# JGI-Bioinformatics/Kmernator

Hardware: AMD Instinct MI355X
Metric: total k-mers/sec at k=31, 150 bp reads (spectrum build, inputs resident in HBM) (higher is better)
Workload: dtype u64

## Files before the change

### kmernator_amd/csrc/kmr_api.hip

```cpp
#include <hip/hip_runtime.h>
#include <dlfcn.h>
#include <unistd.h>
#include <rccl/rccl.h>

#include <algorithm>
#include <atomic>
#include <cmath>
#include <cstdio>
#include <cstdlib>
#include <cstring>
#include <cctype>
#include <memory>
#include <mutex>
#include <string>
#include <type_traits>
#include <vector>

#include "kmr_host.hpp"
#include "kmr_kernels.hpp"
#include "kmr_partition.hpp"
#include "kmr_superkmer.hpp"
#include "kmr_buckets.hpp"
#include "kmr_synth.hpp"
#define KMR_INSTANCES_EXTERN
// ... 1453 lines not shown
		uint32_t dv[2] = {SK_UNI_NONE, 0u};
		HIPCHK(h, hipMemcpy(dv, h->d_uni.get<uint32_t>(), 8, hipMemcpyDeviceToHost));
		if (dv[1]) mixed = true;
		else if (dv[0] != SK_UNI_NONE) { if (w == SK_UNI_NONE) w = dv[0]; else if (w != dv[0]) mixed = true; }
	}
	if (!mixed && w != SK_UNI_NONE) { uni = true; uni_wbits = w; }
	return 0;
}
template <int W> SkLong<W> sk_own_lists(kmr_handle *h, bool refined) {
	SkLong<W> lg{};
	lg.list_first = 0; lg.list_stride = 1;
	if (h->sk_exchange && h->cfg.world_size > 1 && !refined) { lg.list_first = h->cfg.rank; lg.list_stride = h->cfg.world_size; }
	return lg;
}
template <int W> struct SkCountLaunch {
	void (*kern)(PoolView, const uint64_t *, const uint64_t *, uint64_t, uint32_t, CountOut, FinalizeParams, unsigned int *, uint32_t, SkTrackView, SkLong<W>);
	size_t smem;
};
template <int W, int LOG2S, bool TRACK, bool EXT, bool UNI> SkCountLaunch<W> sk_count_form() { return {sk_count_kernel<W, LOG2S, TRACK, EXT, UNI>, sk_count_smem_bytes<W, LOG2S, TRACK, EXT, UNI>()}; }
template <int W> int sk_count_select(kmr_handle *h, bool ext, bool tracking, bool uni, SkCountLaunch<W> &k) {
	k = ext ? sk_count_form<W, COUNT_LOG2S_EXT, false, true, false>() : (tracking ? sk_count_form<W, COUNT_LOG2S, true, false, false>() :
	    (uni ? sk_count_form<W, COUNT_LOG2S, false, false, true>() : sk_count_form<W, COUNT_LOG2S, false, false, false>()));
	const auto kern = k.kern; const size_t smem = k.smem;
	HIPCHK(h, hipFuncSetAttribute((const void *)kern, hipFuncAttributeMaxDynamicSharedMemorySize, (int)smem));
	return 0;
}

template <int W> struct SkFinalize : CountPass {
	bool tracking = false, refined = false, uni = false;
	uint64_t nl = 1; uint64_t *ls = nullptr, *lc = nullptr; uint32_t nch = 0;
	SkTrackView tv{};
	SkLong<W> lgMain{}, lgItems{}; uint64_t n_items = 0;
	uint64_t early_slots = 0; FinalizeCounters early_c{};
};

int sk_refine_lists(kmr_handle *h, uint64_t &nl) {
	const uint32_t fine_bits = h->sk_bits + h->sk_fine_shift;
	const uint64_t nlf = 1ull << fine_bits;
	unsigned int head = 0;
// ... 87 lines not shown
	else { out.wkeys = h->uw_keys.get<uint64_t>(); out.wvals = h->uw_vals.get<uint32_t>(); out.wcap = key_entries(h, h->uw_keys); out.spkt = h->us_pkt.get<uint32_t>(); out.weakCount = wc; }
	out.wcursor = cursors; out.scursor = cursors + 1;
	out.skeys = h->us_keys.get<uint64_t>(); out.sweight = h->us_b8.get<uint8_t>(); out.scap = key_entries(h, h->us_keys);
	out.singCount = sc; out.fc = fc; out.err = h->derr.get<uint32_t>();
	return out;
}
template <int W> int sk_count_pass(kmr_handle *h, SkFinalize<W> &p) {
	const uint64_t nl = p.nl, n_items = p.n_items; const SkTrackView &tv = p.tv;
	uint32_t merge_log2 = 16;
	DevBuf mslots, mext;
	return count_attempts(h, p, [&]() -> int { mslots.reset(); mext.reset(); return 0; }, [&](const CountOut &out, bool repeated, uint32_t &repeat_on) -> int {
		if (repeated) merge_log2 += 3;
		int rc = 0;
		const int grid = (int)std::min<uint64_t>((uint64_t)num_cus(h) * 4, (nl / p.lgMain.list_stride + SK_LBATCH) / SK_LBATCH);
		SkCountLaunch<W> k;
		rc = sk_count_select<W>(h, p.ext, p.tracking, p.uni, k); if (rc) return rc;
		if (p.tracking) HIPCHK(h, hipMemsetAsync(tv.d_unique, 0, 8 * (tv.n + 1), h->stream));
		if (dbg()) { int nb = 0; hipOccupancyMaxActiveBlocksPerMultiprocessor(&nb, (const void *)k.kern, SKC_THREADS, k.smem); fprintf(stderr, "sk_count<W=%d>: %d blocks per CU (LDS %zu), %llu lists, %u chunks\n", W, nb, k.smem, (unsigned long long)nl, p.nch); }
		hipLaunchKernelGGL(k.kern, dim3(grid), dim3(SKC_THREADS), k.smem, h->stream, pool_view(h, h->l1), p.ls, p.lc, nl, h->k, out, p.f, h->work_counter.get<unsigned int>(), sk_dbg_flags("KMR_SK_COUNT_DBG"), tv, p.lgMain);
		HIPCHK(h, hipGetLastError());
		if (!n_items) return 0;
		SkLong<W> &lgItems = p.lgItems;
		if (mslots.alloc(sizeof(Slot<W>) << merge_log2) != hipSuccess) return fail(h, KMR_ERR_OOM, "merge table of the long lists");
		if (p.ext && mext.alloc(sizeof(ExtSlot) << merge_log2) != hipSuccess) return fail(h, KMR_ERR_OOM, "merge table of the long lists");
		hipLaunchKernelGGL(table_clear_kernel<W>, dim3(grid_for(1ull << merge_log2)), dim3(256), 0, h->stream, mslots.get<Slot<W>>(), mext.get<ExtSlot>(), 1ull << merge_log2);
		lgItems.merge.slots = mslots.get<Slot<W>>(); lgItems.merge.ext = mext.get<ExtSlot>(); lgItems.merge.log2cap = merge_log2;
		HIPCHK(h, hipMemsetAsync(lgItems.merge_used, 0, 8, h->stream));
		rc = zero_work_counter(h); if (rc) return rc;
		const int grid2 = (int)std::min<uint64_t>((uint64_t)num_cus(h) * 4, n_items);
		hipLaunchKernelGGL(k.kern, dim3(grid2), dim3(SKC_THREADS), k.smem, h->stream, pool_view(h, h->l1), p.ls, p.lc, nl, h->k, out, p.f, h->work_counter.get<unsigned int>(), sk_dbg_flags("KMR_SK_COUNT_DBG"), tv, lgItems);
		hipLaunchKernelGGL(sk_merge_emit_kernel<W>, dim3(grid_for(1ull << merge_log2)), dim3(256), 0, h->stream, lgItems.merge, out, p.f);
		if (hipGetLastError() != hipSuccess) return fail(h, KMR_ERR_HIP, "long-list launches");
		if (merge_log2 < 30) repeat_on = ERR_TABLE_FULL;
		return 0;
	});
}
template <int W> int sk_append_early(kmr_handle *h, SkFinalize<W> &p) {
	FinalizeCounters &c = p.c; const FinalizeCounters &early_c = p.early_c; unsigned long long *cur = p.cur; const uint64_t early_slots = p.early_slots;
	const size_t eb = 8ull * (W + 1);
	if (cur[0] + early_slots > packed_entries(h, h->ue)) {
		DevBuf bigger;
		HIPCHK(h, bigger.alloc(eb * (cur[0] + early_slots + 4096)));
		HIPCHK(h, hipMemcpyAsync(bigger.get(), h->ue.get(), eb * cur[0], hipMemcpyDeviceToDevice, h->stream)); HIPCHK(h, hipStreamSynchronize(h->stream));
		h->ue = std::move(bigger);
	}
// ... 89 lines not shown
	const SkTrackView tv{};
	SkLong<W> lg = sk_own_lists<W>(h, false);
	lg.long_threshold = h->tune.long_list_chunks ? h->tune.long_list_chunks : 1024;
	uint32_t *sc = nullptr;
	rc = arena_get(h, &sc, h->nb_sing); if (rc) return rc;
	HIPCHK(h, hipMemsetAsync(sc, 0, 4 * h->nb_sing, h->stream));
	CountOut out{};
	out.wentries = h->early.ue.get<uint64_t>(); out.wcursor = h->early.cursor.get<unsigned long long>(); out.wcap = packed_entries(h, h->early.ue);
	out.scursor = h->early.cursor.get<unsigned long long>() + 1;
	out.singCount = sc; out.fc = (FinalizeCounters *)h->early.fc.get(); out.err = h->early.err.get<uint32_t>();
	rc = zero_work_counter(h); if (rc) return rc;
	const uint64_t n_work = hi > lg.list_first ? (hi - lg.list_first + lg.list_stride - 1) / lg.list_stride : 0;
	if (n_work) {
		const int grid = (int)std::min<uint64_t>((uint64_t)num_cus(h) * 4, (n_work + SK_LBATCH) / SK_LBATCH);
		SkCountLaunch<W> k;
		rc = sk_count_select<W>(h, false, false, uni, k); if (rc) return rc;
		TimeSpan t(h, KMR_TIME_COUNT);
		hipLaunchKernelGGL(k.kern, dim3(grid), dim3(SKC_THREADS), k.smem, h->stream, pool_view(h, h->l1), ls, lc, hi, h->k, out, f, h->work_counter.get<unsigned int>(), sk_dbg_flags("KMR_SK_COUNT_DBG"), tv, lg);
		t.end();
		HIPCHK(h, hipGetLastError());
	}
	h->early.active = true; h->early.hi = hi; h->early.min_depth = min_depth;
	return KMR_OK;
}
int count_prefix_superkmer(kmr_handle *h, uint32_t min_depth, uint64_t hi) { return with_w(h, [&](auto W) { return count_prefix_superkmer_t<W()>(h, min_depth, hi); }); }
int finalize_superkmer(kmr_handle *h, uint32_t min_depth) { return with_w(h, [&](auto W) { return finalize_superkmer_t<W()>(h, min_depth); }); }

template <class M> void release(kmr_handle *h) { static_cast<M &>(*h) = M(); }

void free_partition_state(kmr_handle *h) {
	release<BuildMem>(h);
	if (h->tb_copy_stream) { hipStreamDestroy(h->tb_copy_stream); h->tb_copy_stream = nullptr; for (int a = 0; a < 2; a++) { hipEventDestroy(h->tb_ready[a]); hipEventDestroy(h->tb_consumed[a]); h->tb_set_used[a] = false; } }
}

// ... 1226 lines not shown
```

### kmernator_amd/csrc/kmr_instances.hpp

```cpp
#ifndef KMR_INSTANCES_HPP_
#define KMR_INSTANCES_HPP_

#include "kmr_superkmer.hpp"

namespace kmr {

static const int COUNT_LOG2S = 10;
static const int COUNT_LOG2S_EXT = 9;
static const int PD_THREADS = 1024, PD_RPT = 8, PD_LINE = 4;

#ifdef KMR_INSTANCES_EXTERN
#define KMR_T extern template
#else
#define KMR_T template
#endif

#define KMR_SKX(W, WIN, FILT) KMR_T __global__ void sk_extract_kernel<W, WIN, FILT, false>(ReadsView, DevParams, SkParams, PoolView); KMR_T __global__ void sk_extract_kernel<W, WIN, FILT, true>(ReadsView, DevParams, SkParams, PoolView);
#define KMR_SKXL(W, WIN) KMR_T __global__ void sk_extract_lean_kernel<W, WIN, false>(ReadsView, DevParams, SkParams, PoolView, float, SkPacked); KMR_T __global__ void sk_extract_lean_kernel<W, WIN, true>(ReadsView, DevParams, SkParams, PoolView, float, SkPacked);
#define KMR_SKX_W(W) KMR_SKX(W, 16, false) KMR_SKX(W, 16, true) KMR_SKX(W, 8, false) KMR_SKX(W, 8, true) KMR_SKX(W, 4, false) KMR_SKX(W, 4, true) KMR_SKXL(W, 16) KMR_SKXL(W, 8) KMR_SKXL(W, 4)

#define KMR_SKX_W32(W) KMR_SKX(W, 32, false) KMR_SKX(W, 32, true) KMR_SKXL(W, 32)

#define KMR_SKC(W, TRACK) KMR_SKCX(W, TRACK, false)
#define KMR_SKCX(W, TRACK, EXT) KMR_T __global__ void sk_count_kernel<W, EXT ? COUNT_LOG2S_EXT : COUNT_LOG2S, TRACK, EXT>(PoolView, const uint64_t *, const uint64_t *, uint64_t, uint32_t, CountOut, FinalizeParams, unsigned int *, uint32_t, SkTrackView, SkLong<W>);
#define KMR_SKL(W) KMR_T __global__ void sk_lookup_kernel<W>(PoolView, const uint64_t *, const uint64_t *, uint64_t, uint32_t, const uint64_t *, const uint64_t *, const uint32_t *, uint32_t *, uint64_t, unsigned int *, const uint64_t *, const uint64_t *, const uint32_t *, uint64_t, uint64_t);
#define KMR_SKCU(W) KMR_T __global__ void sk_count_kernel<W, COUNT_LOG2S, false, false, true>(PoolView, const uint64_t *, const uint64_t *, uint64_t, uint32_t, CountOut, FinalizeParams, unsigned int *, uint32_t, SkTrackView, SkLong<W>);
#define KMR_SKC_W(W) KMR_SKC(W, false) KMR_SKCU(W) KMR_SKC(W, true) KMR_SKCX(W, false, true) KMR_SKL(W)

#define KMR_EX(W, EXT, OP, SUB) KMR_T __global__ void extract_kernel<W, EXT, OP, SUB>(ReadsView, DevParams, OP);
#define KMR_EX_OP(W, EXT, ...) KMR_T __global__ void extract_kernel<W, EXT, __VA_ARGS__, false>(ReadsView, DevParams, __VA_ARGS__); KMR_T __global__ void extract_kernel<W, EXT, __VA_ARGS__, true>(ReadsView, DevParams, __VA_ARGS__);
#define KMR_EX_W(W) \
	KMR_EX_OP(W, false, InsertOp<W, false>) KMR_EX_OP(W, true, InsertOp<W, true>) \
	KMR_EX_OP(W, false, LinearOp<W, false, false>) KMR_EX_OP(W, false, LinearOp<W, false, true>) \
	KMR_EX_OP(W, true, LinearOp<W, true, false>) KMR_EX_OP(W, true, LinearOp<W, true, true>) \
	KMR_T __global__ void extract_kernel<W, false, LookupOp<W>, false>(ReadsView, DevParams, LookupOp<W>); \
	KMR_T __global__ void extract_kernel<W, false, LookupWeightOp<W>, false>(ReadsView, DevParams, LookupWeightOp<W>);

#define KMR_PD(W, EXT, LEVEL) KMR_T __global__ void partition_direct_kernel<W, EXT, LEVEL, PD_THREADS, PD_RPT, PD_LINE>(PartSource<W>, PoolView, unsigned int *, const int, const int);
#define KMR_OS(W, EXT, REQ) KMR_T __global__ void owner_scatter_kernel<W, EXT, REQ>(const typename PoolRec<W, EXT>::type *, const uint64_t *, const uint32_t *, uint64_t, uint32_t, uint32_t, uint32_t *, uint64_t, unsigned long long *, unsigned int *, uint32_t *, uint32_t *, OwnerFn);
#define KMR_CK(W, EXT, LOG2S, NARROW) KMR_T __global__ void count_kernel<W, EXT, LOG2S, NARROW>(PoolView, const uint64_t *, const uint64_t *, uint64_t, CountOut, FinalizeParams, unsigned int *, int);
#define KMR_PART_W(W) \
	KMR_PD(W, false, 1) KMR_PD(W, false, 2) KMR_PD(W, true, 1) KMR_PD(W, true, 2) \
// ... 34 lines not shown
```

### kmernator_amd/csrc/kmr_superkmer.hpp

```cpp
#ifndef KMR_SUPERKMER_HPP_
#define KMR_SUPERKMER_HPP_

#include "kmr_partition.hpp"
#include "kmr_buckets.hpp"

namespace kmr {

#ifndef KMR_SK_MAX_N
#define KMR_SK_MAX_N 128
#endif
static const uint32_t SK_CHUNK_G = 64;
static const uint32_t SK_MAX_N = KMR_SK_MAX_N;
static const int SK_WAVES = 3;
static const int SK_WINDOW = 16;
static const int SK_RR = 3, SKL_RR = 4;

#ifdef KMR_DEBUG_HOOKS
#define SK_DBG(flags, bit) (((flags) & (bit)) != 0)
#else
#define SK_DBG(flags, bit) false
#endif
struct SkTrackRec { uint32_t raw, good; unsigned long long end_ordinal; };
static const uint32_t SK_TRACK_MAX = 512;
struct SkTrackView { const unsigned long long *bounds; uint32_t n; unsigned int *d_unique, *d_single; };
// ... 1209 lines not shown

static const int SK_STAGE_CHUNKS = 4;
static const int SK_STAGE_G = SK_STAGE_CHUNKS * SK_CHUNK_G;
static const uint32_t SK_LBATCH = 24;
static const uint32_t SK_DESC_CAP = 160;

template <int W> struct SkLong {
	const uint64_t *item_c0, *item_c1;
	uint64_t n_items;
	uint64_t long_threshold;
	uint32_t list_first, list_stride;
	Table<W> merge;
	unsigned long long *merge_used;
};

template <int W, int LOG2S, bool TRACK = false, bool EXT = false, bool UNI = false>
__host__ __device__ constexpr size_t sk_count_smem_bytes() { return (size_t)(1 << LOG2S) * (8 * W + 24 + (W > 1 ? 4 : 0) - (UNI && W > 1 ? 12 : 0) + (TRACK ? 8 : 0) + (EXT ? 28 : 0)) + (size_t)SK_STAGE_G * 16 + 256 + 64 + (TRACK ? 8 * (SK_TRACK_MAX + 1) : 0); }
static const uint64_t SK_EXT_LONG_CHUNKS = 128;
static const int SK_EXT_BLOCKS = 3;
__device__ __forceinline__ uint32_t sk_ext_char(uint32_t code) { return (uint32_t)((0x584e54474341ull >> (8 * code)) & 0xffu); }

#ifndef KMR_SKC_WAVES
#define KMR_SKC_WAVES 4
#endif
static const int SKC_WAVES = KMR_SKC_WAVES, SKC_THREADS = SKC_WAVES * 64;
static const unsigned long long SK_KEY_PENDING = ~0ull;
static const uint32_t SK_ORDERED_FROM = 256;
static const unsigned long long SK_OSLAB = 2048;

template <int W, int LOG2S, bool TRACK = false, bool EXT = false, bool UNI = false>
__global__ __launch_bounds__(SKC_THREADS, EXT ? (W == 1 ? (LOG2S <= 9 ? SK_EXT_BLOCKS : 2) : 1) : ((W == 1 && LOG2S <= 10 && !TRACK) ? 4 : (W == 2 && LOG2S <= 10 && !TRACK ? (UNI ? 4 : 3) : 1)))
void sk_count_kernel(PoolView pool, const uint64_t *list_start, const uint64_t *list_chunks, uint64_t n_lists, uint32_t k,
                     CountOut out, FinalizeParams f, unsigned int *work_counter, uint32_t dbgFlags, SkTrackView tv, SkLong<W> lg) {
	static_assert(!UNI || (!TRACK && !EXT), "the one-weight count pass is the plain one's");
	constexpr int S = 1 << LOG2S;
	constexpr bool LEAN = UNI && W > 1;
#ifndef KMR_SKC_LIMIT_PCT
#define KMR_SKC_LIMIT_PCT 80
#endif
	constexpr uint32_t LIMIT = (uint32_t)(S * (KMR_SKC_LIMIT_PCT / 100.0));
	constexpr int WSLOTS = S / SKC_WAVES;
	extern __shared__ __attribute__((aligned(16))) uint8_t csm[];
	uint64_t *tkeys = (uint64_t *)csm;
	unsigned long long *tcnt = (unsigned long long *)(tkeys + (size_t)S * W);
	double *twsum = (double *)(tcnt + S);
	unsigned long long *tfirst = (unsigned long long *)(twsum + (LEAN ? 0 : S));
	uint32_t *tstate = (uint32_t *)(tfirst + S);
	uint32_t *ttally = tstate + (W > 1 && !LEAN ? S : 0);
	uint32_t *tpkt = ttally + (EXT ? 6 * S : 0);
	uint4 *stage = (uint4 *)(tpkt + (EXT ? S : 0));
	uint8_t *recOf = (uint8_t *)(stage + SK_STAGE_G);
	unsigned long long *tsecond = (unsigned long long *)(csm + (size_t)S * (8 * W + 24 + (W > 1 ? 4 : 0) + (EXT ? 28 : 0)) + (size_t)SK_STAGE_G * 16 + 256 + 64);
	unsigned int *trkU = (unsigned int *)(tsecond + (TRACK ? S : 0)), *trkS = trkU + (SK_TRACK_MAX + 1);
	__shared__ uint32_t s_list, s_sp;
	__shared__ uint32_t s_claimed[2], s_overflow[2];
	__shared__ uint32_t s_stackBits[40], s_stackVal[40];
	__shared__ unsigned long long s_c0[SK_LBATCH + 1], s_c1[SK_LBATCH + 1];
	__shared__ uint32_t s_dchunk[SK_DESC_CAP];
	__shared__ uint8_t s_dcount[SK_DESC_CAP];
	const int t = threadIdx.x, lane = t & 63, wv = t >> 6;
	if (TRACK) for (int i = t; i < 2 * (int)(SK_TRACK_MAX + 1); i += SKC_THREADS) trkU[i] = 0;
	const uint32_t vw = EXT ? 15 : 3;
	unsigned long long uniq = 0, single = 0, keptW = 0, keptS = 0, satK = 0, satS = 0;
	unsigned long long uniqW = 0, singleW = 0;
	unsigned long long wpos = 0, wend = 0, spos = 0, send = 0;
	bool outFull = false;
	if (t == 0) { s_claimed[0] = s_claimed[1] = 0; s_overflow[0] = s_overflow[1] = 0; s_sp = 0; }
	for (int i = t; i < S; i += SKC_THREADS) { tkeys[(size_t)i * W] = EMPTY_KEY; if (W > 1) tkeys[(size_t)i * W + W - 1] = SK_KEY_PENDING; tcnt[i] = 0; if constexpr (!LEAN) twsum[i] = 0.0; tfirst[i] = NO_FIRST; if constexpr (W > 1 && !LEAN) tstate[i] = 0; if (TRACK) tsecond[i] = NO_FIRST; }
	if (EXT) for (int i = t; i < 6 * S; i += SKC_THREADS) ttally[i] = 0;
	lds_barrier();
	const uint32_t singC = f.has_singletons ? (f.min_depth > 1 ? 0u : 2u) : 3u;
	const uint32_t weakMin = ((!f.has_singletons || f.min_depth > 2) && f.min_depth != 1) ? f.min_depth : 0u;
	const uint32_t uniFirst = UNI ? (first_weight_bits(__uint_as_float(f.uni_wbits)) & 0x7fffffu) : 0u;
	const uint4 *poolg = (const uint4 *)pool.base;
	uint4 pre = make_uint4(0, 0, 0, 0); uint32_t preCount = 0; uint64_t preList = ~0ull;
	uint32_t gen = 0;

	const bool itemMode = lg.item_c0 != nullptr;
	const uint32_t grab = itemMode ? 1u : SK_LBATCH;
	for (;;) {
		if (t == 0) s_list = atomicAdd(work_counter, grab);
		lds_barrier();
		const uint64_t lfirst = s_list;
		const uint64_t stride = lg.list_stride ? lg.list_stride : 1u;
		const uint64_t n_work = itemMode ? lg.n_items : (n_lists > lg.list_first ? (n_lists - lg.list_first + stride - 1) / stride : 0);
		if (lfirst >= n_work) break;
		const uint32_t nl = (uint32_t)(n_work - lfirst < (uint64_t)grab ? n_work - lfirst : (uint64_t)grab);
		if ((uint32_t)t < nl) {
			uint64_t a, b;
			if (itemMode) { a = lg.item_c0[lfirst + t]; b = lg.item_c1[lfirst + t]; }
			else { const uint64_t l = lg.list_first + (lfirst + t) * stride; a = list_start[l]; b = list_start[l + 1]; if (lg.long_threshold && b - a > lg.long_threshold) b = a; }
			s_c0[t] = a; s_c1[t] = b;
		}
		lds_barrier();
// ... 74 lines not shown
#pragma unroll
						for (int wi = 0; wi < W; wi++) {
							const uint32_t d0 = up ? win[2 * wi + 1] : win[2 * wi], d1 = up ? win[2 * wi + 2] : win[2 * wi + 1], d2 = up ? win[2 * wi + 3] : win[2 * wi + 2];
							const uint32_t hi = (uint32_t)(((((uint64_t)d0) << 32 | d1) << r) >> 32), lo = (uint32_t)(((((uint64_t)d1) << 32 | d2) << r) >> 32);
							kf.w[wi] = ((uint64_t)hi << 32) | lo;
						}
						uint32_t rcIn = 0; uint64_t kfFirst = 0;
						if constexpr (EXT) {
							kfFirst = kf.w[0];
							if ((k >> 5) < (uint32_t)W) { uint64_t wsel = kf.w[0];
#pragma unroll
								for (int wi = 1; wi < W; wi++) if ((k >> 5) == (uint32_t)wi) wsel = kf.w[wi];
								rcIn = (uint32_t)(wsel >> (62u - 2u * (k & 31u))) & 3u; }
							else { const uint32_t b = j + k; rcIn = (((const uint32_t *)(wstage + rs + 1))[b >> 4] >> (30 - 2 * (b & 15u))) & 3u; }
						}
						key_clip_tail<W>(kf, k);
						st.key = key_canonical<W>(kf, k, st.fwd);
						const uint64_t h = slot_hash<W>(st.key.w);
						st.slot = (uint32_t)(h >> (64 - LOG2S));
						st.step = ((uint32_t)(h >> (64 - 2 * LOG2S)) & (uint32_t)(S - 1)) | 1u;
						st.mine = ((uint32_t)(h >> 20) & subMask) == val;
						if constexpr (!UNI) st.w = uniformW ? hw : ww[j];
						st.ord = ord0 + j;
						if constexpr (EXT) {
							uint32_t lc = j > 0 ? leftCarry : sk_hdr_ext_left(hy), rc = sk_hdr_ext_right(hy);
							if (j + 1 < n) rc = rcIn;
							leftCarry = (uint32_t)(kfFirst >> 62);
							const uint32_t q2 = ((const uint16_t *)xq)[j];
							uint32_t lq = q2 & 0xffu, rq = q2 >> 8;
							if (!st.fwd) {
								const uint32_t tl = rc < 4u ? 3u - rc : rc, tr = lc < 4u ? 3u - lc : lc, tq = rq;
								lc = tl; rc = tr; rq = lq; lq = tq;
							}
							st.x = lc | (rc << 8) | (lq << 16) | (rq << 24);
						}
					};
					if (left) {
						enter_record(); seed_window();
						if (EXT && j > 0) { const uint32_t b = j - 1; leftCarry = (((const uint32_t *)(wstage + rs + 1))[b >> 4] >> (30 - 2 * (b & 15u))) & 3u; }
						prepare(kA);
					}
					uint32_t dbgSink = 0;
					auto step_one = [&](KState &cur, KState &nxt) {
						if (left) {
							uint32_t s = cur.slot;
							const float wa = __uint_as_float(UNI ? f.uni_wbits : cur.w);
							unsigned long long old = EMPTY_KEY;
							const bool tableOn = !SK_DBG(dbgFlags, 1) && cur.mine;
							if (W == 1 || padded) { if (tableOn) old = atomicCAS((unsigned long long *)&tkeys[(size_t)s * W], (unsigned long long)EMPTY_KEY, (unsigned long long)cur.key.w[0]); }
							j++; left--; sb += 2;
							if (left) {
								if (j >= n) {
									rs = rs + sk_hdr_granules(hy);
									{ const uint32_t g0 = rs < SK_CHUNK_G - 1 ? rs : SK_CHUNK_G - 1; const uint4 hh = wstage[g0]; hx = hh.x; hy = hh.y; hw = hh.w; }
									j = 0;
									seed_window();
									enter_record();
								} else if (sb > 62u) seed_window();
								prepare(nxt);
							}
							if (SK_DBG(dbgFlags, 1)) { dbgSink ^= (uint32_t)cur.key.w[0] ^ s; }
// ... 61 lines not shown
									}
									s = (s + cur.step) & (S - 1);
								}
								if (!placed) s_overflow[fl] = 1;
								else {
									atomicAdd(&tcnt[s], 1ull | ((unsigned long long)(cur.fwd ? 1 : 0) << 32));
									if constexpr (!UNI) atomicAdd(&twsum[s], (double)wa);
									const unsigned long long fp = UNI ? (((unsigned long long)cur.ord << FIRST_ORD_SHIFT) | ((unsigned long long)(cur.fwd ? 1u : 0u) << 23) | (unsigned long long)uniFirst) : first_pack(cur.ord, cur.fwd, wa);
									if (TRACK) {
										const unsigned long long was = atomicMin(&tfirst[s], fp);
										const unsigned long long cand = was > fp ? was : fp;
										if (cand != NO_FIRST) atomicMin(&tsecond[s], cand);
									} else atomicMin(&tfirst[s], fp);
									if constexpr (EXT) {
										const uint32_t lc = cur.x & 0xffu, rc = (cur.x >> 8) & 0xffu, lq = (cur.x >> 16) & 0xffu, rq = cur.x >> 24;
										if (lq >= f.ext_min_q || lc > 3u) atomicAdd(&ttally[(size_t)s * 6 + (lc >> 1)], 1u << (16 * (lc & 1u)));
										if (rq >= f.ext_min_q || rc > 3u) atomicAdd(&ttally[(size_t)s * 6 + 3 + (rc >> 1)], 1u << (16 * (rc & 1u)));
										if (claimedHere != claimedBefore) tpkt[s] = sk_ext_char(lc) | (sk_ext_char(rc) << 8) | (cur.x & 0xffff0000u);
									}
								}
							}
						}
					};
					for (uint32_t it = 0; it < Lk; it += 2) { step_one(kA, kB); step_one(kB, kA); }
					if (SK_DBG(dbgFlags, 1) && dbgSink == 0x12345u) s_overflow[fl] = 2;
					claimedHere = (uint32_t)__builtin_amdgcn_readlane((int)sk_wave_scan_u32(claimedHere), 63);
					if (lane == 0 && claimedHere) atomicAdd(&s_claimed[fl], claimedHere);
					sk_wave_lds_order();
					cur = nxt; curCount = nxtCount;
				}
				if (wantPre && lj + 1 < nl) { const uint64_t n0 = s_c0[lj + 1], n1 = s_c1[lj + 1]; if (n0 + wv < n1) { fetch(n0 + wv, pre, preCount); preList = lfirst + lj + 1; } }
			};
// ... 19 lines not shown
					nsel += (uint32_t)__builtin_popcountll(nm);
				}
				sk_wave_lds_order();
#pragma unroll 1
				for (uint32_t sb0 = 0; sb0 < nsel; sb0 += 64) {
					const bool used = sb0 + (uint32_t)lane < nsel;
					const int s = used ? (int)wsel[sb0 + lane] : wv * WSLOTS;
					const unsigned long long cf = used ? tcnt[s] : 0ull;
					const uint32_t count = (uint32_t)cf;
					uint32_t cls = !used ? 0u : ((count == 1 && singC != 3u) ? singC : (count < weakMin ? 0u : 1u));
					if (SK_DBG(dbgFlags, 2)) cls = 0;
					Key<W> key;
#pragma unroll
					for (int q = 0; q < W; q++) key.w[q] = used ? tkeys[(size_t)s * W + q] : 0ull;
					const unsigned long long fst = used ? tfirst[s] : NO_FIRST;
					const double wsum = UNI ? (double)count * (double)__uint_as_float(f.uni_wbits) : (used ? twsum[s] : 0.0);
					if (TRACK && used) {
						auto behind = [&](unsigned long long ord) -> uint32_t {
							uint32_t lo = 0, hi = tv.n;
							while (lo < hi) { const uint32_t mid = (lo + hi) >> 1; if (tv.bounds[mid] <= ord) lo = mid + 1; else hi = mid; }
							return lo;
						};
						const uint32_t iu = behind(fst >> 24);
						atomicAdd(&trkU[iu], 1u);
						atomicAdd(&trkS[iu], 1u);
						const unsigned long long sec = tsecond[s];
						if (sec != NO_FIRST) atomicAdd(&trkS[behind(sec >> 24)], 0xffffffffu);
					}
					if (itemMode) {
						cls = 0;
						for (int turn = 0; turn < (W == 1 ? 1 : 64); turn++) {
// ... 9 lines not shown
									atomicMin(&sl->first, fst);
									if constexpr (EXT) {
										ExtSlot *es = &lg.merge.ext[ms];
#pragma unroll
										for (int j = 0; j < 12; j++) { const uint32_t v = (ttally[(size_t)s * 6 + (j >> 1)] >> (16 * (j & 1))) & 0xffffu; if (v) atomicAdd(&es->tally[j], v); }
										es->pkt = tpkt[s];
									}
								}
							}
						}
					}
					const unsigned long long mw = __ballot(cls == 1), ms = __ballot(cls == 2);
					if (mw) {
						const uint32_t cnt = (uint32_t)__builtin_popcountll(mw);
						if (wpos + cnt > wend) {
							for (unsigned long long e = wpos + lane; e < wend && e < out.wcap; e += 64) { if (out.wentries) out.wentries[e * (W + 1) + W] = 0; else out.wvals[e * vw] = 0; }
							unsigned long long g = 0;
							if (lane == 0) g = atomicAdd(out.wcursor, SK_OSLAB);
							wpos = ((unsigned long long)(uint32_t)__shfl((int)(g >> 32), 0, 64) << 32) | (uint32_t)__shfl((int)(uint32_t)g, 0, 64);
							wend = wpos + SK_OSLAB;
							if (wend > out.wcap) { if (lane == 0) atomicOr(out.err, (uint32_t)ERR_ENTRIES_FULL); outFull = true; wend = wpos; }
						}
						if (!outFull) {
							if (cls == 1) {
								const uint64_t pos = wpos + (uint32_t)__builtin_popcountll(mw & below);
								uint32_t fwdc = (uint32_t)(cf >> 32), cnt16 = count;
								if (f.has_singletons && first_forward(fst)) fwdc -= 1;
								if (cnt16 >= SK_ORDERED_FROM) { satK++; satS += count; if (cnt16 > 65535u) { cnt16 = 65535u; if (fwdc > 65534u) fwdc = 65534u; } }
								if (fwdc > 65535u) fwdc = 65535u;
								const uint32_t wbits = __float_as_uint((float)(f.has_singletons ? wsum + first_weight_shift(fst) : wsum));
								if (out.wentries) {
									uint64_t ew[W + 1];
#pragma unroll
									for (int q = 0; q < W; q++) ew[q] = key.w[q];
									ew[W] = bb_pack_value(cnt16, wbits, fwdc);
									bb_store_entry<W>(out.wentries, pos, ew);
								} else {
#pragma unroll
									for (int q = 0; q < W; q++) out.wkeys[pos * W + q] = key.w[q];
									uint32_t *v = out.wvals + pos * vw;
									v[0] = cnt16; v[1] = wbits; v[2] = fwdc;
									if constexpr (EXT) {
#pragma unroll
										for (int j = 0; j < 12; j++) v[3 + j] = (ttally[(size_t)s * 6 + (j >> 1)] >> (16 * (j & 1))) & 0xffffu;
									}
								}
							}
							wpos += cnt; keptW += lane == 0 ? cnt : 0u;
						}
					}
					if (out.weakCount) {
						const uint64_t bucket = cls == 1 ? key_hash<W>(key, f.kb) & (f.nb_weak - 1) : 0;
						bucket_count_add(out.weakCount, bucket, cls == 1 && !outFull);
					}
					if (ms) {
						const uint32_t cnt = (uint32_t)__builtin_popcountll(ms);
						if (spos + cnt > send) {
							for (unsigned long long e = spos + lane; e < send && e < out.scap; e += 64) out.sweight[e] = 0;
							unsigned long long g = 0;
							if (lane == 0) g = atomicAdd(out.scursor, SK_OSLAB);
							spos = ((unsigned long long)(uint32_t)__shfl((int)(g >> 32), 0, 64) << 32) | (uint32_t)__shfl((int)(uint32_t)g, 0, 64);
							send = spos + SK_OSLAB;
							if (send > out.scap) { if (lane == 0) atomicOr(out.err, (uint32_t)ERR_ENTRIES_FULL); outFull = true; send = spos; }
						}
						uint64_t bucket = 0;
						if (!outFull && cls == 2) {
							const uint64_t pos = spos + (uint32_t)__builtin_popcountll(ms & below);
							bucket = key_hash<W>(key, f.kb) & (f.nb_sing - 1);
#pragma unroll
							for (int q = 0; q < W; q++) out.skeys[pos * W + q] = key.w[q];
							const float wf = (float)wsum;
							out.sweight[pos] = (uint8_t)((unsigned char)(((double)wf * 254.0)) + 1);
							if constexpr (EXT) out.spkt[pos] = tpkt[s];
						}
						bucket_count_add(out.singCount, bucket, cls == 2 && !outFull);
						if (!outFull) { spos += cnt; keptS += lane == 0 ? cnt : 0u; }
					}
				}
				sk_wave_lds_order();
#pragma unroll
				for (int i = 0; i < WSLOTS / 64; i++) {
					const int s = wv * WSLOTS + i * 64 + lane;
					if ((usedMask[i] >> lane) & 1ull) {
						tkeys[(size_t)s * W] = EMPTY_KEY; if (W > 1) tkeys[(size_t)s * W + W - 1] = SK_KEY_PENDING; tcnt[s] = 0; if constexpr (!LEAN) twsum[s] = 0.0; tfirst[s] = NO_FIRST; if constexpr (W > 1 && !LEAN) tstate[s] = 0; if (TRACK) tsecond[s] = NO_FIRST;
						if constexpr (EXT) {
#pragma unroll
							for (int q = 0; q < 6; q++) ttally[(size_t)s * 6 + q] = 0;
						}
					}
				}
			};
			auto clear_table = [&]() {
				for (int i = t; i < S; i += SKC_THREADS) { tkeys[(size_t)i * W] = EMPTY_KEY; if (W > 1) tkeys[(size_t)i * W + W - 1] = SK_KEY_PENDING; tcnt[i] = 0; if constexpr (!LEAN) twsum[i] = 0.0; tfirst[i] = NO_FIRST; if constexpr (W > 1 && !LEAN) tstate[i] = 0; if (TRACK) tsecond[i] = NO_FIRST; }
				if (EXT) for (int i = t; i < 6 * S; i += SKC_THREADS) ttally[i] = 0;
			};

			insert_pass(0, 0, true);
			lds_barrier();
			const bool ovf = s_overflow[fl] != 0 || s_claimed[fl] > LIMIT;
			if (t == 0) { s_claimed[fl ^ 1u] = 0; s_overflow[fl ^ 1u] = 0; }
			if (!ovf) {
				emit_pass();
				lds_barrier();
				continue;
			}
			clear_table();
			if (t == 0) { s_sp = 2; s_stackBits[0] = 1; s_stackVal[0] = 0; s_stackBits[1] = 1; s_stackVal[1] = 1; }
			lds_barrier();
// ... 12 lines not shown
						else {
							s_stackBits[s_sp] = bits + 1; s_stackVal[s_sp] = val; s_sp++;
							s_stackBits[s_sp] = bits + 1; s_stackVal[s_sp] = val | (1u << bits); s_sp++;
						}
					}
					lds_barrier();
					continue;
				}
				emit_pass();
				lds_barrier();
			}
			if (t == 0) { s_claimed[0] = s_claimed[1] = 0; s_overflow[0] = s_overflow[1] = 0; }
			lds_barrier();
		}
	}
	for (unsigned long long e = wpos + lane; e < wend && e < out.wcap; e += 64) { if (out.wentries) out.wentries[e * (W + 1) + W] = 0; else out.wvals[e * vw] = 0; }
	for (unsigned long long e = spos + lane; e < send && e < out.scap; e += 64) out.sweight[e] = 0;
	uniq = wave_sum(uniq) + uniqW; single = wave_sum(single) + singleW; satK = wave_sum(satK); satS = wave_sum(satS);
	if (lane == 0) {
		if (uniq) atomicAdd(&out.fc->unique, uniq); if (single) atomicAdd(&out.fc->singletons, single);
		if (keptW) atomicAdd(&out.fc->weak_kept, keptW); if (keptS) atomicAdd(&out.fc->sing_kept, keptS);
		if (satK) { atomicAdd(&out.fc->saturated, satK); atomicAdd(&out.fc->sat_sightings, satS); }
	}
	if (TRACK) {
		lds_barrier();
		for (uint32_t i = (uint32_t)t; i <= tv.n && i <= SK_TRACK_MAX; i += SKC_THREADS) { if (trkU[i]) atomicAdd(&tv.d_unique[i], trkU[i]); if (trkS[i]) atomicAdd(&tv.d_single[i], trkS[i]); }
	}
}


template <int W>
__global__ __launch_bounds__(256)
void sk_merge_emit_kernel(Table<W> tbl, CountOut out, FinalizeParams f) {
	const uint32_t vw = tbl.ext ? 15 : 3;
	const uint32_t singC = f.has_singletons ? (f.min_depth > 1 ? 0u : 2u) : 3u;
	const uint32_t weakMin = ((!f.has_singletons || f.min_depth > 2) && f.min_depth != 1) ? f.min_depth : 0u;
	const uint64_t cap = 1ull << tbl.log2cap;
	unsigned long long uniq = 0, single = 0, keptW = 0, keptS = 0;
// ... 497 lines not shown
```

Before: 58.10 billion.

## Slim sk_count kernel arguments and specialize item mode and output format at compile time

```diff
diff --git a/kmernator_amd/csrc/kmr_api.hip b/kmernator_amd/csrc/kmr_api.hip
--- a/kmernator_amd/csrc/kmr_api.hip
+++ b/kmernator_amd/csrc/kmr_api.hip
@@ -1491,15 +1491,30 @@
 	return lg;
 }
 template <int W> struct SkCountLaunch {
-	void (*kern)(PoolView, const uint64_t *, const uint64_t *, uint64_t, uint32_t, CountOut, FinalizeParams, unsigned int *, uint32_t, SkTrackView, SkLong<W>);
+	void (*kern)(const uint4 *, const uint64_t *, const uint64_t *, uint64_t, uint32_t, SkCountHot, unsigned int *, uint32_t, const SkCountArgs<W> *);
 	size_t smem;
 };
-template <int W, int LOG2S, bool TRACK, bool EXT, bool UNI> SkCountLaunch<W> sk_count_form() { return {sk_count_kernel<W, LOG2S, TRACK, EXT, UNI>, sk_count_smem_bytes<W, LOG2S, TRACK, EXT, UNI>()}; }
-template <int W> int sk_count_select(kmr_handle *h, bool ext, bool tracking, bool uni, SkCountLaunch<W> &k) {
-	k = ext ? sk_count_form<W, COUNT_LOG2S_EXT, false, true, false>() : (tracking ? sk_count_form<W, COUNT_LOG2S, true, false, false>() :
-	    (uni ? sk_count_form<W, COUNT_LOG2S, false, false, true>() : sk_count_form<W, COUNT_LOG2S, false, false, false>()));
+template <int W, int LOG2S, bool TRACK, bool EXT, bool UNI, bool ITEM> SkCountLaunch<W> sk_count_form() { return {sk_count_kernel<W, LOG2S, TRACK, EXT, UNI, ITEM>, sk_count_smem_bytes<W, LOG2S, TRACK, EXT, UNI>()}; }
+template <int W, bool ITEM> SkCountLaunch<W> sk_count_forms(bool ext, bool tracking, bool uni) {
+	if constexpr (!ITEM) { if (tracking && !ext) return sk_count_form<W, COUNT_LOG2S, true, false, false, false>(); }
+	return ext ? sk_count_form<W, COUNT_LOG2S_EXT, false, true, false, ITEM>() :
+	    (uni ? sk_count_form<W, COUNT_LOG2S, false, false, true, ITEM>() : sk_count_form<W, COUNT_LOG2S, false, false, false, ITEM>());
+}
+template <int W> int sk_count_select(kmr_handle *h, bool ext, bool tracking, bool uni, bool item, const CountOut &out, const SkLong<W> &lg, SkCountLaunch<W> &k) {
+	if (item && tracking) return fail(h, KMR_ERR_STATE, "internal: the size tracker's count pass has no long-list items");
+	if (item != (lg.item_c0 != nullptr) || (item && (!lg.item_c1 || !lg.merge.slots || !lg.merge_used))) return fail(h, KMR_ERR_STATE, "internal: count pass and its work items disagree");
+	if (ext ? (!out.wkeys || !out.wvals || !out.weakCount) : !out.wentries) return fail(h, KMR_ERR_STATE, "internal: count pass and its entry buffers disagree");
+	k = item ? sk_count_forms<W, true>(ext, tracking, uni) : sk_count_forms<W, false>(ext, tracking, uni);
 	const auto kern = k.kern; const size_t smem = k.smem;
 	HIPCHK(h, hipFuncSetAttribute((const void *)kern, hipFuncAttributeMaxDynamicSharedMemorySize, (int)smem));
+	return 0;
+}
+template <int W> int sk_count_launch(kmr_handle *h, const SkCountLaunch<W> &k, int grid, const uint64_t *ls, const uint64_t *lc, uint64_t nl, const CountOut &out, const FinalizeParams &f, const SkTrackView &tv, const SkLong<W> &lg) {
+	SkCountArgs<W> a{out, f, tv, lg};
+	SkCountArgs<W> *d = nullptr;
+	int rc = arena_get(h, &d, 1); if (rc) return rc;
+	hipLaunchKernelGGL(sk_count_args_kernel<W>, dim3(1), dim3(64), 0, h->stream, a, d);
+	hipLaunchKernelGGL(k.kern, dim3(grid), dim3(SKC_THREADS), k.smem, h->stream, (const uint4 *)pool_view(h, h->l1).base, ls, lc, nl, h->k, sk_count_hot<W>(a), h->work_counter.get<unsigned int>(), sk_dbg_flags("KMR_SK_COUNT_DBG"), (const SkCountArgs<W> *)d);
 	return 0;
 }
 
@@ -1617,10 +1632,10 @@
 		int rc = 0;
 		const int grid = (int)std::min<uint64_t>((uint64_t)num_cus(h) * 4, (nl / p.lgMain.list_stride + SK_LBATCH) / SK_LBATCH);
 		SkCountLaunch<W> k;
-		rc = sk_count_select<W>(h, p.ext, p.tracking, p.uni, k); if (rc) return rc;
+		rc = sk_count_select<W>(h, p.ext, p.tracking, p.uni, false, out, p.lgMain, k); if (rc) return rc;
 		if (p.tracking) HIPCHK(h, hipMemsetAsync(tv.d_unique, 0, 8 * (tv.n + 1), h->stream));
 		if (dbg()) { int nb = 0; hipOccupancyMaxActiveBlocksPerMultiprocessor(&nb, (const void *)k.kern, SKC_THREADS, k.smem); fprintf(stderr, "sk_count<W=%d>: %d blocks per CU (LDS %zu), %llu lists, %u chunks\n", W, nb, k.smem, (unsigned long long)nl, p.nch); }
-		hipLaunchKernelGGL(k.kern, dim3(grid), dim3(SKC_THREADS), k.smem, h->stream, pool_view(h, h->l1), p.ls, p.lc, nl, h->k, out, p.f, h->work_counter.get<unsigned int>(), sk_dbg_flags("KMR_SK_COUNT_DBG"), tv, p.lgMain);
+		rc = sk_count_launch<W>(h, k, grid, p.ls, p.lc, nl, out, p.f, tv, p.lgMain); if (rc) return rc;
 		HIPCHK(h, hipGetLastError());
 		if (!n_items) return 0;
 		SkLong<W> &lgItems = p.lgItems;
@@ -1631,7 +1646,8 @@
 		HIPCHK(h, hipMemsetAsync(lgItems.merge_used, 0, 8, h->stream));
 		rc = zero_work_counter(h); if (rc) return rc;
 		const int grid2 = (int)std::min<uint64_t>((uint64_t)num_cus(h) * 4, n_items);
-		hipLaunchKernelGGL(k.kern, dim3(grid2), dim3(SKC_THREADS), k.smem, h->stream, pool_view(h, h->l1), p.ls, p.lc, nl, h->k, out, p.f, h->work_counter.get<unsigned int>(), sk_dbg_flags("KMR_SK_COUNT_DBG"), tv, lgItems);
+		rc = sk_count_select<W>(h, p.ext, p.tracking, p.uni, true, out, lgItems, k); if (rc) return rc;
+		rc = sk_count_launch<W>(h, k, grid2, p.ls, p.lc, nl, out, p.f, tv, lgItems); if (rc) return rc;
 		hipLaunchKernelGGL(sk_merge_emit_kernel<W>, dim3(grid_for(1ull << merge_log2)), dim3(256), 0, h->stream, lgItems.merge, out, p.f);
 		if (hipGetLastError() != hipSuccess) return fail(h, KMR_ERR_HIP, "long-list launches");
 		if (merge_log2 < 30) repeat_on = ERR_TABLE_FULL;
@@ -1751,10 +1767,11 @@
 	if (n_work) {
 		const int grid = (int)std::min<uint64_t>((uint64_t)num_cus(h) * 4, (n_work + SK_LBATCH) / SK_LBATCH);
 		SkCountLaunch<W> k;
-		rc = sk_count_select<W>(h, false, false, uni, k); if (rc) return rc;
+		rc = sk_count_select<W>(h, false, false, uni, false, out, lg, k); if (rc) return rc;
 		TimeSpan t(h, KMR_TIME_COUNT);
-		hipLaunchKernelGGL(k.kern, dim3(grid), dim3(SKC_THREADS), k.smem, h->stream, pool_view(h, h->l1), ls, lc, hi, h->k, out, f, h->work_counter.get<unsigned int>(), sk_dbg_flags("KMR_SK_COUNT_DBG"), tv, lg);
+		rc = sk_count_launch<W>(h, k, grid, ls, lc, hi, out, f, tv, lg);
 		t.end();
+		if (rc) return rc;
 		HIPCHK(h, hipGetLastError());
 	}
 	h->early.active = true; h->early.hi = hi; h->early.min_depth = min_depth;
diff --git a/kmernator_amd/csrc/kmr_instances.hpp b/kmernator_amd/csrc/kmr_instances.hpp
--- a/kmernator_amd/csrc/kmr_instances.hpp
+++ b/kmernator_amd/csrc/kmr_instances.hpp
@@ -22,10 +22,12 @@
 #define KMR_SKX_W32(W) KMR_SKX(W, 32, false) KMR_SKX(W, 32, true) KMR_SKXL(W, 32)
 
 #define KMR_SKC(W, TRACK) KMR_SKCX(W, TRACK, false)
-#define KMR_SKCX(W, TRACK, EXT) KMR_T __global__ void sk_count_kernel<W, EXT ? COUNT_LOG2S_EXT : COUNT_LOG2S, TRACK, EXT>(PoolView, const uint64_t *, const uint64_t *, uint64_t, uint32_t, CountOut, FinalizeParams, unsigned int *, uint32_t, SkTrackView, SkLong<W>);
+#define KMR_SKCI(W, TRACK, EXT, UNI, ITEM) KMR_T __global__ void sk_count_kernel<W, EXT ? COUNT_LOG2S_EXT : COUNT_LOG2S, TRACK, EXT, UNI, ITEM>(const uint4 *, const uint64_t *, const uint64_t *, uint64_t, uint32_t, SkCountHot, unsigned int *, uint32_t, const SkCountArgs<W> *);
+#define KMR_SKCX(W, TRACK, EXT) KMR_SKCI(W, TRACK, EXT, false, false)
 #define KMR_SKL(W) KMR_T __global__ void sk_lookup_kernel<W>(PoolView, const uint64_t *, const uint64_t *, uint64_t, uint32_t, const uint64_t *, const uint64_t *, const uint32_t *, uint32_t *, uint64_t, unsigned int *, const uint64_t *, const uint64_t *, const uint32_t *, uint64_t, uint64_t);
-#define KMR_SKCU(W) KMR_T __global__ void sk_count_kernel<W, COUNT_LOG2S, false, false, true>(PoolView, const uint64_t *, const uint64_t *, uint64_t, uint32_t, CountOut, FinalizeParams, unsigned int *, uint32_t, SkTrackView, SkLong<W>);
-#define KMR_SKC_W(W) KMR_SKC(W, false) KMR_SKCU(W) KMR_SKC(W, true) KMR_SKCX(W, false, true) KMR_SKL(W)
+#define KMR_SKCU(W) KMR_SKCI(W, false, false, true, false)
+#define KMR_SKC_W(W) KMR_SKC(W, false) KMR_SKCU(W) KMR_SKC(W, true) KMR_SKCX(W, false, true) \
+	KMR_SKCI(W, false, false, false, true) KMR_SKCI(W, false, false, true, true) KMR_SKCI(W, false, true, false, true) KMR_SKL(W)
 
 #define KMR_EX(W, EXT, OP, SUB) KMR_T __global__ void extract_kernel<W, EXT, OP, SUB>(ReadsView, DevParams, OP);
 #define KMR_EX_OP(W, EXT, ...) KMR_T __global__ void extract_kernel<W, EXT, __VA_ARGS__, false>(ReadsView, DevParams, __VA_ARGS__); KMR_T __global__ void extract_kernel<W, EXT, __VA_ARGS__, true>(ReadsView, DevParams, __VA_ARGS__);
diff --git a/kmernator_amd/csrc/kmr_superkmer.hpp b/kmernator_amd/csrc/kmr_superkmer.hpp
--- a/kmernator_amd/csrc/kmr_superkmer.hpp
+++ b/kmernator_amd/csrc/kmr_superkmer.hpp
@@ -1247,8 +1247,19 @@
 	unsigned long long *merge_used;
 };
 
+struct SkCountHot {
+	uint64_t *wout;
+	uint32_t *wvals; unsigned long long *wcursor; uint64_t wcap;
+	uint32_t min_depth, has_singletons, uni_wbits, ext_min_q;
+};
+template <int W> struct SkCountArgs { CountOut out; FinalizeParams f; SkTrackView tv; SkLong<W> lg; };
+template <int W> __host__ inline SkCountHot sk_count_hot(const SkCountArgs<W> &a) {
+	return {a.out.wentries ? a.out.wentries : a.out.wkeys, a.out.wvals, a.out.wcursor, a.out.wcap, a.f.min_depth, a.f.has_singletons, a.f.uni_wbits, a.f.ext_min_q};
+}
+template <int W> __global__ void sk_count_args_kernel(SkCountArgs<W> a, SkCountArgs<W> *dst) { if (threadIdx.x == 0 && blockIdx.x == 0) *dst = a; }
+
 template <int W, int LOG2S, bool TRACK = false, bool EXT = false, bool UNI = false>
-__host__ __device__ constexpr size_t sk_count_smem_bytes() { return (size_t)(1 << LOG2S) * (8 * W + 24 + (W > 1 ? 4 : 0) - (UNI && W > 1 ? 12 : 0) + (TRACK ? 8 : 0) + (EXT ? 28 : 0)) + (size_t)SK_STAGE_G * 16 + 256 + 64 + (TRACK ? 8 * (SK_TRACK_MAX + 1) : 0); }
+__host__ __device__ constexpr size_t sk_count_smem_bytes() { return (size_t)(1 << LOG2S) * (8 * W + 24 + (W > 1 ? 4 : 0) - (UNI ? 8 : 0) - (UNI && W > 1 ? 4 : 0) + (TRACK ? 8 : 0) + (EXT ? 28 : 0)) + (size_t)SK_STAGE_G * 16 + 256 + 64 + (TRACK ? 8 * (SK_TRACK_MAX + 1) : 0); }
 static const uint64_t SK_EXT_LONG_CHUNKS = 128;
 static const int SK_EXT_BLOCKS = 3;
 __device__ __forceinline__ uint32_t sk_ext_char(uint32_t code) { return (uint32_t)((0x584e54474341ull >> (8 * code)) & 0xffu); }
@@ -1261,13 +1272,17 @@
 static const uint32_t SK_ORDERED_FROM = 256;
 static const unsigned long long SK_OSLAB = 2048;
 
-template <int W, int LOG2S, bool TRACK = false, bool EXT = false, bool UNI = false>
+template <int W, int LOG2S, bool TRACK = false, bool EXT = false, bool UNI = false, bool ITEM = false>
 __global__ __launch_bounds__(SKC_THREADS, EXT ? (W == 1 ? (LOG2S <= 9 ? SK_EXT_BLOCKS : 2) : 1) : ((W == 1 && LOG2S <= 10 && !TRACK) ? 4 : (W == 2 && LOG2S <= 10 && !TRACK ? (UNI ? 4 : 3) : 1)))
-void sk_count_kernel(PoolView pool, const uint64_t *list_start, const uint64_t *list_chunks, uint64_t n_lists, uint32_t k,
-                     CountOut out, FinalizeParams f, unsigned int *work_counter, uint32_t dbgFlags, SkTrackView tv, SkLong<W> lg) {
+void sk_count_kernel(const uint4 *poolg, const uint64_t *list_start, const uint64_t *list_chunks, uint64_t n_lists, uint32_t k,
+                     SkCountHot hot, unsigned int *work_counter, uint32_t dbgFlags, const SkCountArgs<W> *__restrict__ args) {
+	const CountOut &out = args->out; const FinalizeParams &f = args->f; const SkTrackView &tv = args->tv; const SkLong<W> &lg = args->lg;
 	static_assert(!UNI || (!TRACK && !EXT), "the one-weight count pass is the plain one's");
 	constexpr int S = 1 << LOG2S;
 	constexpr bool LEAN = UNI && W > 1;
+	constexpr bool WSUM = !UNI;
+	constexpr bool PACKED = !EXT;
+	static_assert(!ITEM || !TRACK, "the size tracker's pass has no long-list items");
 #ifndef KMR_SKC_LIMIT_PCT
 #define KMR_SKC_LIMIT_PCT 80
 #endif
@@ -1277,7 +1292,7 @@
 	uint64_t *tkeys = (uint64_t *)csm;
 	unsigned long long *tcnt = (unsigned long long *)(tkeys + (size_t)S * W);
 	double *twsum = (double *)(tcnt + S);
-	unsigned long long *tfirst = (unsigned long long *)(twsum + (LEAN ? 0 : S));
+	unsigned long long *tfirst = (unsigned long long *)(twsum + (WSUM ? S : 0));
 	uint32_t *tstate = (uint32_t *)(tfirst + S);
 	uint32_t *ttally = tstate + (W > 1 && !LEAN ? S : 0);
 	uint32_t *tpkt = ttally + (EXT ? 6 * S : 0);
@@ -1287,6 +1302,7 @@
 	unsigned int *trkU = (unsigned int *)(tsecond + (TRACK ? S : 0)), *trkS = trkU + (SK_TRACK_MAX + 1);
 	__shared__ uint32_t s_list, s_sp;
 	__shared__ uint32_t s_claimed[2], s_overflow[2];
+	__shared__ unsigned long long s_sat[2];
 	__shared__ uint32_t s_stackBits[40], s_stackVal[40];
 	__shared__ unsigned long long s_c0[SK_LBATCH + 1], s_c1[SK_LBATCH + 1];
 	__shared__ uint32_t s_dchunk[SK_DESC_CAP];
@@ -1294,23 +1310,21 @@
 	const int t = threadIdx.x, lane = t & 63, wv = t >> 6;
 	if (TRACK) for (int i = t; i < 2 * (int)(SK_TRACK_MAX + 1); i += SKC_THREADS) trkU[i] = 0;
 	const uint32_t vw = EXT ? 15 : 3;
-	unsigned long long uniq = 0, single = 0, keptW = 0, keptS = 0, satK = 0, satS = 0;
-	unsigned long long uniqW = 0, singleW = 0;
+	unsigned long long uniqW = 0, singleW = 0, keptW = 0, keptS = 0;
 	unsigned long long wpos = 0, wend = 0, spos = 0, send = 0;
 	bool outFull = false;
-	if (t == 0) { s_claimed[0] = s_claimed[1] = 0; s_overflow[0] = s_overflow[1] = 0; s_sp = 0; }
-	for (int i = t; i < S; i += SKC_THREADS) { tkeys[(size_t)i * W] = EMPTY_KEY; if (W > 1) tkeys[(size_t)i * W + W - 1] = SK_KEY_PENDING; tcnt[i] = 0; if constexpr (!LEAN) twsum[i] = 0.0; tfirst[i] = NO_FIRST; if constexpr (W > 1 && !LEAN) tstate[i] = 0; if (TRACK) tsecond[i] = NO_FIRST; }
+	if (t == 0) { s_claimed[0] = s_claimed[1] = 0; s_overflow[0] = s_overflow[1] = 0; s_sp = 0; s_sat[0] = s_sat[1] = 0; }
+	for (int i = t; i < S; i += SKC_THREADS) { tkeys[(size_t)i * W] = EMPTY_KEY; if (W > 1) tkeys[(size_t)i * W + W - 1] = SK_KEY_PENDING; tcnt[i] = 0; if constexpr (WSUM) twsum[i] = 0.0; tfirst[i] = NO_FIRST; if constexpr (W > 1 && !LEAN) tstate[i] = 0; if (TRACK) tsecond[i] = NO_FIRST; }
 	if (EXT) for (int i = t; i < 6 * S; i += SKC_THREADS) ttally[i] = 0;
 	lds_barrier();
-	const uint32_t singC = f.has_singletons ? (f.min_depth > 1 ? 0u : 2u) : 3u;
-	const uint32_t weakMin = ((!f.has_singletons || f.min_depth > 2) && f.min_depth != 1) ? f.min_depth : 0u;
-	const uint32_t uniFirst = UNI ? (first_weight_bits(__uint_as_float(f.uni_wbits)) & 0x7fffffu) : 0u;
-	const uint4 *poolg = (const uint4 *)pool.base;
+	const uint32_t singC = hot.has_singletons ? (hot.min_depth > 1 ? 0u : 2u) : 3u;
+	const uint32_t weakMin = ((!hot.has_singletons || hot.min_depth > 2) && hot.min_depth != 1) ? hot.min_depth : 0u;
+	const uint32_t uniFirst = UNI ? (first_weight_bits(__uint_as_float(hot.uni_wbits)) & 0x7fffffu) : 0u;
 	uint4 pre = make_uint4(0, 0, 0, 0); uint32_t preCount = 0; uint64_t preList = ~0ull;
 	uint32_t gen = 0;
 
-	const bool itemMode = lg.item_c0 != nullptr;
-	const uint32_t grab = itemMode ? 1u : SK_LBATCH;
+	constexpr bool itemMode = ITEM;
+	constexpr uint32_t grab = itemMode ? 1u : SK_LBATCH;
 	for (;;) {
 		if (t == 0) s_list = atomicAdd(work_counter, grab);
 		lds_barrier();
@@ -1415,8 +1429,19 @@
 								rcIn = (uint32_t)(wsel >> (62u - 2u * (k & 31u))) & 3u; }
 							else { const uint32_t b = j + k; rcIn = (((const uint32_t *)(wstage + rs + 1))[b >> 4] >> (30 - 2 * (b & 15u))) & 3u; }
 						}
-						key_clip_tail<W>(kf, k);
-						st.key = key_canonical<W>(kf, k, st.fwd);
+						if constexpr (W == 1) {
+							const uint32_t padBits = 64u - 2u * k;
+							kf.w[0] &= ~0ull << padBits;
+							uint32_t rh = __builtin_bitreverse32((uint32_t)kf.w[0]), rl = __builtin_bitreverse32((uint32_t)(kf.w[0] >> 32));
+							rh = ((rh >> 1) & 0x55555555u) | ((rh & 0x55555555u) << 1);
+							rl = ((rl >> 1) & 0x55555555u) | ((rl & 0x55555555u) << 1);
+							const uint64_t kr = (((uint64_t)~rh << 32) | (uint32_t)~rl) << padBits;
+							st.fwd = kf.w[0] <= kr;
+							st.key.w[0] = st.fwd ? kf.w[0] : kr;
+						} else {
+							key_clip_tail<W>(kf, k);
+							st.key = key_canonical<W>(kf, k, st.fwd);
+						}
 						const uint64_t h = slot_hash<W>(st.key.w);
 						st.slot = (uint32_t)(h >> (64 - LOG2S));
 						st.step = ((uint32_t)(h >> (64 - 2 * LOG2S)) & (uint32_t)(S - 1)) | 1u;
@@ -1445,7 +1470,7 @@
 					auto step_one = [&](KState &cur, KState &nxt) {
 						if (left) {
 							uint32_t s = cur.slot;
-							const float wa = __uint_as_float(UNI ? f.uni_wbits : cur.w);
+							const float wa = __uint_as_float(UNI ? hot.uni_wbits : cur.w);
 							unsigned long long old = EMPTY_KEY;
 							const bool tableOn = !SK_DBG(dbgFlags, 1) && cur.mine;
 							if (W == 1 || padded) { if (tableOn) old = atomicCAS((unsigned long long *)&tkeys[(size_t)s * W], (unsigned long long)EMPTY_KEY, (unsigned long long)cur.key.w[0]); }
@@ -1537,8 +1562,8 @@
 									} else atomicMin(&tfirst[s], fp);
 									if constexpr (EXT) {
 										const uint32_t lc = cur.x & 0xffu, rc = (cur.x >> 8) & 0xffu, lq = (cur.x >> 16) & 0xffu, rq = cur.x >> 24;
-										if (lq >= f.ext_min_q || lc > 3u) atomicAdd(&ttally[(size_t)s * 6 + (lc >> 1)], 1u << (16 * (lc & 1u)));
-										if (rq >= f.ext_min_q || rc > 3u) atomicAdd(&ttally[(size_t)s * 6 + 3 + (rc >> 1)], 1u << (16 * (rc & 1u)));
+										if (lq >= hot.ext_min_q || lc > 3u) atomicAdd(&ttally[(size_t)s * 6 + (lc >> 1)], 1u << (16 * (lc & 1u)));
+										if (rq >= hot.ext_min_q || rc > 3u) atomicAdd(&ttally[(size_t)s * 6 + 3 + (rc >> 1)], 1u << (16 * (rc & 1u)));
 										if (claimedHere != claimedBefore) tpkt[s] = sk_ext_char(lc) | (sk_ext_char(rc) << 8) | (cur.x & 0xffff0000u);
 									}
 								}
@@ -1588,7 +1613,7 @@
 #pragma unroll
 					for (int q = 0; q < W; q++) key.w[q] = used ? tkeys[(size_t)s * W + q] : 0ull;
 					const unsigned long long fst = used ? tfirst[s] : NO_FIRST;
-					const double wsum = UNI ? (double)count * (double)__uint_as_float(f.uni_wbits) : (used ? twsum[s] : 0.0);
+					const double wsum = UNI ? (double)count * (double)__uint_as_float(hot.uni_wbits) : (used ? twsum[s] : 0.0);
 					if (TRACK && used) {
 						auto behind = [&](unsigned long long ord) -> uint32_t {
 							uint32_t lo = 0, hi = tv.n;
@@ -1628,31 +1653,31 @@
 					if (mw) {
 						const uint32_t cnt = (uint32_t)__builtin_popcountll(mw);
 						if (wpos + cnt > wend) {
-							for (unsigned long long e = wpos + lane; e < wend && e < out.wcap; e += 64) { if (out.wentries) out.wentries[e * (W + 1) + W] = 0; else out.wvals[e * vw] = 0; }
+							for (unsigned long long e = wpos + lane; e < wend && e < hot.wcap; e += 64) { if (PACKED) hot.wout[e * (W + 1) + W] = 0; else hot.wvals[e * vw] = 0; }
 							unsigned long long g = 0;
-							if (lane == 0) g = atomicAdd(out.wcursor, SK_OSLAB);
+							if (lane == 0) g = atomicAdd(hot.wcursor, SK_OSLAB);
 							wpos = ((unsigned long long)(uint32_t)__shfl((int)(g >> 32), 0, 64) << 32) | (uint32_t)__shfl((int)(uint32_t)g, 0, 64);
 							wend = wpos + SK_OSLAB;
-							if (wend > out.wcap) { if (lane == 0) atomicOr(out.err, (uint32_t)ERR_ENTRIES_FULL); outFull = true; wend = wpos; }
+							if (wend > hot.wcap) { if (lane == 0) atomicOr(out.err, (uint32_t)ERR_ENTRIES_FULL); outFull = true; wend = wpos; }
 						}
 						if (!outFull) {
 							if (cls == 1) {
 								const uint64_t pos = wpos + (uint32_t)__builtin_popcountll(mw & below);
 								uint32_t fwdc = (uint32_t)(cf >> 32), cnt16 = count;
-								if (f.has_singletons && first_forward(fst)) fwdc -= 1;
-								if (cnt16 >= SK_ORDERED_FROM) { satK++; satS += count; if (cnt16 > 65535u) { cnt16 = 65535u; if (fwdc > 65534u) fwdc = 65534u; } }
+								if (hot.has_singletons && first_forward(fst)) fwdc -= 1;
+								if (cnt16 >= SK_ORDERED_FROM) { atomicAdd(&s_sat[0], 1ull); atomicAdd(&s_sat[1], (unsigned long long)count); if (cnt16 > 65535u) { cnt16 = 65535u; if (fwdc > 65534u) fwdc = 65534u; } }
 								if (fwdc > 65535u) fwdc = 65535u;
-								const uint32_t wbits = __float_as_uint((float)(f.has_singletons ? wsum + first_weight_shift(fst) : wsum));
-								if (out.wentries) {
+								const uint32_t wbits = __float_as_uint((float)(hot.has_singletons ? wsum + first_weight_shift(fst) : wsum));
+								if constexpr (PACKED) {
 									uint64_t ew[W + 1];
 #pragma unroll
 									for (int q = 0; q < W; q++) ew[q] = key.w[q];
 									ew[W] = bb_pack_value(cnt16, wbits, fwdc);
-									bb_store_entry<W>(out.wentries, pos, ew);
+									bb_store_entry<W>(hot.wout, pos, ew);
 								} else {
 #pragma unroll
-									for (int q = 0; q < W; q++) out.wkeys[pos * W + q] = key.w[q];
-									uint32_t *v = out.wvals + pos * vw;
+									for (int q = 0; q < W; q++) hot.wout[pos * W + q] = key.w[q];
+									uint32_t *v = hot.wvals + pos * vw;
 									v[0] = cnt16; v[1] = wbits; v[2] = fwdc;
 									if constexpr (EXT) {
 #pragma unroll
@@ -1660,10 +1685,10 @@
 									}
 								}
 							}
-							wpos += cnt; keptW += lane == 0 ? cnt : 0u;
+							wpos += cnt; keptW += cnt;
 						}
 					}
-					if (out.weakCount) {
+					if constexpr (!PACKED) {
 						const uint64_t bucket = cls == 1 ? key_hash<W>(key, f.kb) & (f.nb_weak - 1) : 0;
 						bucket_count_add(out.weakCount, bucket, cls == 1 && !outFull);
 					}
@@ -1688,7 +1713,7 @@
 							if constexpr (EXT) out.spkt[pos] = tpkt[s];
 						}
 						bucket_count_add(out.singCount, bucket, cls == 2 && !outFull);
-						if (!outFull) { spos += cnt; keptS += lane == 0 ? cnt : 0u; }
+						if (!outFull) { spos += cnt; keptS += cnt; }
 					}
 				}
 				sk_wave_lds_order();
@@ -1696,7 +1721,7 @@
 				for (int i = 0; i < WSLOTS / 64; i++) {
 					const int s = wv * WSLOTS + i * 64 + lane;
 					if ((usedMask[i] >> lane) & 1ull) {
-						tkeys[(size_t)s * W] = EMPTY_KEY; if (W > 1) tkeys[(size_t)s * W + W - 1] = SK_KEY_PENDING; tcnt[s] = 0; if constexpr (!LEAN) twsum[s] = 0.0; tfirst[s] = NO_FIRST; if constexpr (W > 1 && !LEAN) tstate[s] = 0; if (TRACK) tsecond[s] = NO_FIRST;
+						tkeys[(size_t)s * W] = EMPTY_KEY; if (W > 1) tkeys[(size_t)s * W + W - 1] = SK_KEY_PENDING; tcnt[s] = 0; if constexpr (WSUM) twsum[s] = 0.0; tfirst[s] = NO_FIRST; if constexpr (W > 1 && !LEAN) tstate[s] = 0; if (TRACK) tsecond[s] = NO_FIRST;
 						if constexpr (EXT) {
 #pragma unroll
 							for (int q = 0; q < 6; q++) ttally[(size_t)s * 6 + q] = 0;
@@ -1705,7 +1730,7 @@
 				}
 			};
 			auto clear_table = [&]() {
-				for (int i = t; i < S; i += SKC_THREADS) { tkeys[(size_t)i * W] = EMPTY_KEY; if (W > 1) tkeys[(size_t)i * W + W - 1] = SK_KEY_PENDING; tcnt[i] = 0; if constexpr (!LEAN) twsum[i] = 0.0; tfirst[i] = NO_FIRST; if constexpr (W > 1 && !LEAN) tstate[i] = 0; if (TRACK) tsecond[i] = NO_FIRST; }
+				for (int i = t; i < S; i += SKC_THREADS) { tkeys[(size_t)i * W] = EMPTY_KEY; if (W > 1) tkeys[(size_t)i * W + W - 1] = SK_KEY_PENDING; tcnt[i] = 0; if constexpr (WSUM) twsum[i] = 0.0; tfirst[i] = NO_FIRST; if constexpr (W > 1 && !LEAN) tstate[i] = 0; if (TRACK) tsecond[i] = NO_FIRST; }
 				if (EXT) for (int i = t; i < 6 * S; i += SKC_THREADS) ttally[i] = 0;
 			};
 
@@ -1748,14 +1773,13 @@
 			lds_barrier();
 		}
 	}
-	for (unsigned long long e = wpos + lane; e < wend && e < out.wcap; e += 64) { if (out.wentries) out.wentries[e * (W + 1) + W] = 0; else out.wvals[e * vw] = 0; }
+	for (unsigned long long e = wpos + lane; e < wend && e < hot.wcap; e += 64) { if (PACKED) hot.wout[e * (W + 1) + W] = 0; else hot.wvals[e * vw] = 0; }
 	for (unsigned long long e = spos + lane; e < send && e < out.scap; e += 64) out.sweight[e] = 0;
-	uniq = wave_sum(uniq) + uniqW; single = wave_sum(single) + singleW; satK = wave_sum(satK); satS = wave_sum(satS);
 	if (lane == 0) {
-		if (uniq) atomicAdd(&out.fc->unique, uniq); if (single) atomicAdd(&out.fc->singletons, single);
+		if (uniqW) atomicAdd(&out.fc->unique, uniqW); if (singleW) atomicAdd(&out.fc->singletons, singleW);
 		if (keptW) atomicAdd(&out.fc->weak_kept, keptW); if (keptS) atomicAdd(&out.fc->sing_kept, keptS);
-		if (satK) { atomicAdd(&out.fc->saturated, satK); atomicAdd(&out.fc->sat_sightings, satS); }
-	}
+	}
+	if (t == 0 && s_sat[0]) { atomicAdd(&out.fc->saturated, s_sat[0]); atomicAdd(&out.fc->sat_sightings, s_sat[1]); }
 	if (TRACK) {
 		lds_barrier();
 		for (uint32_t i = (uint32_t)t; i <= tv.n && i <= SK_TRACK_MAX; i += SKC_THREADS) { if (trkU[i]) atomicAdd(&tv.d_unique[i], trkU[i]); if (trkS[i]) atomicAdd(&tv.d_single[i], trkS[i]); }
```

Result: faster. 60.55 billion (median of 6 runs) (+4.2%).
